# amisr/volumetricinterp

Hardware: AMD Instinct MI355X
Metric: fit+eval timesteps/sec (higher is better)
Workload: dtype f64

## Files before the change

### include/vinterp.h

```cpp
#ifndef VINTERP_H
#define VINTERP_H

#include <stddef.h>
#include <stdint.h>

#ifdef __cplusplus
extern "C" {
#endif

#define VI_ABI_VERSION 2

typedef enum vi_status {
    VI_OK = 0,
    VI_ERR_INVALID = -1,
    VI_ERR_HIP = -2,
    VI_ERR_ROCBLAS = -3,
    VI_ERR_ROCSOLVER = -4,
    VI_ERR_NOMEM = -5,
    VI_ERR_UNSUPPORTED = -6,
    VI_ERR_RCCL = -7
} vi_status;

typedef struct vi_ctx vi_ctx;
typedef struct vi_model vi_model;
// ... 65 lines not shown
int  vi_eval_track_f64(vi_model* model, int64_t Q, const double* d_lat, const double* d_lon, const double* d_alt,
                       const int32_t* d_rec, const double* d_w, int64_t R, const double* d_C,
                       const double* d_hull_eq, int32_t F, double hull_tol, double* d_out);
int  vi_eval_track_grad_f64(vi_model* model, int64_t Q, const double* d_lat, const double* d_lon, const double* d_alt,
                            const int32_t* d_rec, const double* d_w, int64_t R, const double* d_C,
                            const double* d_hull_eq, int32_t F, double hull_tol, int32_t frame, double* d_out);
int  vi_eval_slant_f64(vi_model* model, int64_t P, const double* d_a, const double* d_b, const int32_t* d_rec, const double* d_w,
                       int64_t R, const double* d_C, const double* d_hull_eq, int32_t F, double hull_tol, int32_t n,
                       const double* d_x, const double* d_wq, double* d_out, double* d_chord);
int  vi_eval_slant_basis_f64(vi_model* model, int64_t P, const double* d_a, const double* d_b, const double* d_hull_eq, int32_t F,
                             double hull_tol, int32_t n, const double* d_x, const double* d_wq, double* d_Y, double* d_chord);
int  vi_eval_basis_f64(vi_model* model, int64_t Q, const double* d_lat, const double* d_lon, const double* d_alt,
                       const double* d_hull_eq, int32_t F, double hull_tol, double* d_Y);
int  vi_eval_resident_f64(vi_model* model, int64_t Q, int64_t T, const double* d_Y, const double* d_C, double* d_out);
enum { VI_FRAME_MODEL = 0, VI_FRAME_ENU = 1 };
int  vi_eval_grad_basis_f64(vi_model* model, int64_t Q, const double* d_lat, const double* d_lon, const double* d_alt,
                            const double* d_hull_eq, int32_t F, double hull_tol, int32_t frame, double* d_G);
int  vi_eval_resident_err_f64(vi_model* model, int64_t Q, int64_t T, const double* d_Y, const double* d_dC, double* d_out);
int  vi_eval_resident_err_at_f64(vi_model* model, int64_t outer, int64_t L, int64_t inner, int64_t T, const double* d_Y,
                                 const double* d_dC, const int32_t* d_idx, double* d_out);
int  vi_eval_records_err_f64(vi_model* model, int64_t Q, const double* d_Y, const int32_t* d_rec, const double* d_w, int64_t R,
                             const double* d_dC, double* d_out);
int  vi_eval_track_err_f64(vi_model* model, int64_t Q, const double* d_lat, const double* d_lon, const double* d_alt,
                           const int32_t* d_rec, const double* d_w, int64_t R, const double* d_dC,
                           const double* d_hull_eq, int32_t F, double hull_tol, double* d_out);
int  vi_eval_slant_err_f64(vi_model* model, int64_t P, const double* d_a, const double* d_b, const int32_t* d_rec, const double* d_w,
                           int64_t R, const double* d_dC, const double* d_hull_eq, int32_t F, double hull_tol, int32_t n,
                           const double* d_x, const double* d_wq, double* d_out, double* d_chord);
int  vi_eval_resident_gradcov_f64(vi_model* model, int64_t Q, int64_t T, const double* d_G, const double* d_dC, double* d_out);
int  vi_eval_grad_cov_f64(vi_model* model, int64_t Q, const double* d_lat, const double* d_lon, const double* d_alt,
                          const double* d_dC, const double* d_hull_eq, int32_t F, double hull_tol, int32_t frame, double* d_out);
int  vi_eval_records_gradcov_f64(vi_model* model, int64_t Q, const double* d_G, const int32_t* d_rec, const double* d_w, int64_t R,
                                 const double* d_dC, double* d_out);
int  vi_eval_track_grad_cov_f64(vi_model* model, int64_t Q, const double* d_lat, const double* d_lon, const double* d_alt,
                                const int32_t* d_rec, const double* d_w, int64_t R, const double* d_dC,
                                const double* d_hull_eq, int32_t F, double hull_tol, int32_t frame, double* d_out);
int  vi_eval_hess_f64(vi_model* model, int64_t Q, const double* d_lat, const double* d_lon, const double* d_alt,
                      const double* d_C, const double* d_hull_eq, int32_t F, double hull_tol, int32_t frame, double* d_out);
int  vi_eval_hess_basis_f64(vi_model* model, int64_t Q, const double* d_lat, const double* d_lon, const double* d_alt,
                            const double* d_hull_eq, int32_t F, double hull_tol, int32_t frame, double* d_H);
int  vi_eval_peak_f64(vi_model* model, int64_t T, int64_t Q, const double* d_lat, const double* d_lon, const double* d_h0,
                      const double* d_lo, const double* d_hi, const double* d_C, const double* d_hull_eq, int32_t F,
                      double hull_tol, int32_t kind, int32_t max_iter, double tol, double* d_out, int32_t* d_status,
                      int32_t* d_iter);
int  vi_eval_level_f64(vi_model* model, int64_t T, int64_t Q, const double* d_lat, const double* d_lon, const double* d_ends,
                       const double* d_level, const double* d_C, const double* d_hull_eq, int32_t F, double hull_tol,
                       int32_t max_iter, double tol, double* d_out, int32_t* d_status, int32_t* d_iter);
int  vi_eval_ray_peak_f64(vi_model* model, int64_t T, int64_t P, const double* d_a, const double* d_b, const double* d_start,
                          const double* d_lo, const double* d_hi, const double* d_C, const double* d_hull_eq, int32_t F,
                          double hull_tol, int32_t kind, int32_t max_iter, double tol, double* d_out, int32_t* d_status,
                          int32_t* d_iter);
int  vi_eval_ray_level_f64(vi_model* model, int64_t T, int64_t P, const double* d_a, const double* d_b, const double* d_ends,
                           const double* d_level, const double* d_C, const double* d_hull_eq, int32_t F, double hull_tol,
                           int32_t max_iter, double tol, double* d_out, int32_t* d_status, int32_t* d_iter);
int  vi_eval_extremum_f64(vi_model* model, int64_t T, int64_t P, const double* d_x0, const double* d_radius, const double* d_C,
                          const double* d_hull_eq, int32_t F, double hull_tol, int32_t kind, double max_step, int32_t max_iter,
                          double tol, double* d_out, int32_t* d_status, int32_t* d_iter);
int    vi_eval_resident_peak_f64(vi_model* model, int64_t outer, int64_t L, int64_t inner, int64_t T, const double* d_Y,
                                 const double* d_C, int32_t kind, double* d_val, int32_t* d_idx, void* d_work, size_t work_bytes);
size_t vi_eval_resident_peak_work_bytes(vi_model* model, int64_t outer, int64_t L, int64_t inner, int64_t T);
int    vi_reduce_basis_f64(vi_model* model, int64_t outer, int64_t L, int64_t inner, const double* d_Y, const double* d_w,
                           double* d_Yr);
int    vi_eval_resident_cross_f64(vi_model* model, int64_t outer, int64_t L, int64_t inner, int64_t T, const double* d_Y,
                                  const double* d_C, const double* d_level, int32_t which, int32_t direction, int32_t* d_idx,
                                  void* d_work, size_t work_bytes);
int  vi_model_set_eval_precision(vi_model* model, int32_t chain_f32);
int  vi_ctx_set_eval_timing(vi_ctx* ctx, int32_t on);
int  vi_eval_kernel_ms(vi_ctx* ctx, double* ms);
int  vi_solve_timing(vi_ctx* ctx, int enable, int64_t* launches, int64_t* systems, int64_t* timed,
                     double* total_ms, double* max_ms);
int  vi_solve_rounds(vi_ctx* ctx, int64_t* rounds);
int  vi_eval_f64_host(vi_model* model, int64_t Q, const double* h_lat, const double* h_lon,
                      const double* h_alt, int64_t T, const double* h_C,
                      const double* h_hull_eq, int32_t F, double hull_tol, double* h_out);

int  vi_host_alloc(size_t bytes, void** out);
int  vi_host_free(void* p);

int  vi_normal_eq_f64(vi_ctx* ctx, int64_t T, int64_t P, int32_t N, const double* d_At,
                      const double* d_W, const double* d_b, double* d_AWA, double* d_y);

int  vi_form_system_f64(vi_ctx* ctx, int64_t B, int32_t N, const double* d_AWA, const int32_t* d_rec,
                        const double* d_alpha, const double* d_R, double* d_X);

int  vi_solve_trunc_f64(vi_ctx* ctx, int64_t B, int32_t N, double* d_X, const double* d_y,
                        const int32_t* d_rec, double rcond, double* d_C, int32_t* d_rank,
                        double pinv_rcond, double* d_H );

int  vi_chi2_f64(vi_ctx* ctx, int64_t B, int64_t P, int32_t N, const double* d_At, const double* d_C,
                 const int32_t* d_rec, const double* d_W, const double* d_b, double* d_chi2);

int  vi_cov_f64(vi_ctx* ctx, int64_t T, int32_t N, const double* d_H, const double* d_AWA, double* d_dC);

int  vi_warm_prepare_f64(vi_ctx* ctx, int64_t B, int32_t N, const double* d_AWA, const int32_t* d_rec,
                         const double* d_alpha0, const double* d_R, const double* d_y, double rcond,
                         double* d_C, int32_t* d_rank, double* d_V, double* d_D1, double* d_D2, double* d_yt);
int  vi_warm_solve_f64(vi_ctx* ctx, int64_t B, int32_t N, const double* d_D1, const double* d_D2,
                       const double* d_yt, const double* d_V, const int32_t* d_slot, const double* d_alpha,
                       double rcond, double* d_C, int32_t* d_rank, int32_t* d_sweeps );
int  vi_max_sweeps(void);

size_t vi_rotation_log_bytes(int32_t N);
int  vi_decompose_f64(vi_ctx* ctx, int64_t B, int32_t N, const double* d_AWA, const int32_t* d_rec,
                      const double* d_alpha0, const double* d_R, const double* d_y, double rcond, double* d_C,
                      int32_t* d_rank, void* d_log, int32_t* d_nround);
int  vi_warm_finish_f64(vi_ctx* ctx, int64_t B, int32_t N, const void* d_log, const int32_t* d_nround,
                        const double* d_AWA, const int32_t* d_rec, const double* d_R, const double* d_y,
                        double* d_V, double* d_D1, double* d_D2, double* d_yt);

int  vi_warm_rebase_f64(vi_ctx* ctx, int64_t B, int64_t nplain, int32_t N, const double* d_AWA, const double* d_R,
                        const double* d_y, const int32_t* d_rec, const int32_t* d_slot, const double* d_alpha, double rcond,
                        double* d_V, double* d_D1, double* d_D2, double* d_yt, double* d_C, int32_t* d_rank,
                        int32_t* d_sweeps );

int  vi_reg_floor_f64(vi_ctx* ctx, int64_t T, int32_t N, const double* d_AWA, const double* d_R, double* d_out);

int  vi_basis_solve_f64(vi_ctx* ctx, int64_t B, int32_t N, const double* d_AWA, const double* d_y,
                        const int32_t* d_rec, const int32_t* d_basis, const double* d_alpha, const double* d_V,
                        const double* d_D2, double rcond, double* d_C, int32_t* d_rank, int32_t* d_sweeps );

int  vi_warm_chi2_one_f64(vi_ctx* ctx, int32_t N, int64_t P, const double* d_D1, const double* d_D2,
                          const double* d_yt, const double* d_V, int32_t slot, double alpha, double rcond,
                          const double* d_At, int32_t rec, const double* d_W, const double* d_b,
                          double* d_scratch, double* h_chi2);

int  vi_brent_warm_f64(vi_ctx* ctx, int64_t ntask, int32_t N, int64_t P, double* d_D1, double* d_D2, double* d_yt,
                       double* d_V, const double* d_AWA, const double* d_R, const double* d_y, const double* h_rebase,
                       const double* d_At, const double* d_W, const double* d_b,
                       const int32_t* d_rec, const int32_t* d_slot, const double* d_xa, const double* d_xb,
                       const double* d_fa, const double* d_fb, const double* d_nu, double rcond, double* d_root,
                       double* d_other, int32_t* d_iters, int32_t* d_funcalls, int32_t* d_status);
int  vi_brent_warm_supported(int32_t N, int64_t P);
int  vi_brent_host_one_f64(vi_ctx* ctx, int32_t N, int64_t P, double* d_D1, double* d_D2, double* d_yt, double* d_V,
                           const double* d_AWA, const double* d_R, const double* d_y, const double* h_rebase,
                           const double* d_At, const double* d_W, const double* d_b, int32_t rec, int32_t slot,
                           double xa, double xb, double fa, double fb, double nu, double rcond, double* d_scratch,
                           double* h_out);
int  vi_exp10_f64(const double* x, double* out, int64_t n);

int  vi_gcv_terms_f64(vi_ctx* ctx, int64_t np, int64_t P, int32_t N, const double* d_At, const int32_t* d_pidx,
                      const double* d_AWA, const double* d_y, const double* d_W, const double* d_b,
                      double alpha, const double* d_R, double rcond, double* d_res);

int  vi_rccl_unique_id(char* out128);
int  vi_rccl_init(vi_ctx* ctx, int nranks, int rank, const char* id128);
int  vi_rccl_bcast_f64(vi_ctx* ctx, double* d_buf, int64_t count, int root);
int  vi_rccl_destroy(vi_ctx* ctx);

int  vi_eigvals_f64(vi_ctx* ctx, int64_t B, int32_t N, double* d_X, double* d_lam, int32_t* d_sweeps);

int  vi_qr_similarity_f64(vi_ctx* ctx, int64_t B, int32_t N, const double* d_X, const double* d_y, double* d_X1,
                          double* d_y1, double* d_Q);

int  vi_walk_form_f64(vi_ctx* ctx, int64_t B, int32_t N, const double* d_AWA, const int32_t* d_rec, const double* d_V,
                      const double* d_D2, const int32_t* d_basis, const double* d_y, const double* d_alpha, double* d_X,
                      double* d_scl, double* d_yt);

#ifdef __cplusplus
}
#endif
#endif
```

### volumetricinterp_amd/csrc/vi_qr.hip

```cpp
#include "vi_common.h"
#include "vi_solver.h"

#include <type_traits>

#ifdef VI_STAMPS
__device__ unsigned long long g_qr_stamps[8];
#define QR_STAMP(k)                                                        \
    do {                                                                   \
        const unsigned long long t_ = __builtin_readcyclecounter();        \
        if (blockIdx.x == 0 && threadIdx.x == 0) g_qr_stamps[k] += t_ - stamp_t; \
        stamp_t = __builtin_readcyclecounter();                            \
    } while (0)
#else
#define QR_STAMP(k)
#endif

namespace {

template <int CTRL, int ROWMASK>
__device__ __forceinline__ double dpp_mov(double v)
{
    const int lo = __builtin_amdgcn_update_dpp(__double2loint(v), __double2loint(v), CTRL, ROWMASK, 0xf, false);
    const int hi = __builtin_amdgcn_update_dpp(__double2hiint(v), __double2hiint(v), CTRL, ROWMASK, 0xf, false);
    return __hiloint2double(hi, lo);
}
__device__ __forceinline__ double octet_sum(double v)
{
    v += dpp_mov<0xB1, 0xf>(v);
    v += dpp_mov<0x4E, 0xf>(v);
    v += dpp_mov<0x141, 0xf>(v);
    return v;
}
__device__ __forceinline__ double wave_max_octets(double v)
{
    v = fmax(v, dpp_mov<0x118, 0xf>(v));
    v = fmax(v, dpp_mov<0x142, 0xa>(v));
    v = fmax(v, dpp_mov<0x143, 0xc>(v));
    const int lo = __builtin_amdgcn_readlane(__double2loint(v), 63);
    const int hi = __builtin_amdgcn_readlane(__double2hiint(v), 63);
    return __hiloint2double(hi, lo);
}
__device__ __forceinline__ double wave_sum(double v)
{
    v += dpp_mov<0xB1, 0xf>(v);
    v += dpp_mov<0x4E, 0xf>(v);
    v += dpp_mov<0x141, 0xf>(v);
    v += dpp_mov<0x140, 0xf>(v);
    {
        const int lo = __builtin_amdgcn_update_dpp(0, __double2loint(v), 0x142, 0xa, 0xf, false);
        const int hi = __builtin_amdgcn_update_dpp(0, __double2hiint(v), 0x142, 0xa, 0xf, false);
        v += __hiloint2double(hi, lo);
    }
    {
        const int lo = __builtin_amdgcn_update_dpp(0, __double2loint(v), 0x143, 0xc, 0xf, false);
        const int hi = __builtin_amdgcn_update_dpp(0, __double2hiint(v), 0x143, 0xc, 0xf, false);
        v += __hiloint2double(hi, lo);
    }
    const int lo = __builtin_amdgcn_readlane(__double2loint(v), 63);
    const int hi = __builtin_amdgcn_readlane(__double2hiint(v), 63);
    return __hiloint2double(hi, lo);
}

__device__ __forceinline__ void lds_barrier()
{
    asm volatile("s_waitcnt lgkmcnt(0)\n\ts_barrier" ::: "memory");
}

__device__ __forceinline__ double qr_rsqrt(double x)
{
    const double y = __builtin_amdgcn_rsq(x);
    const double e = fma(-x * y, y, 1.0);
    return fma(y, e * fma(0.375, e, 0.5), y);
}
__device__ __forceinline__ double qr_rcp(double x)
{
    double y = __builtin_amdgcn_rcp(x);
    y = fma(y, fma(-x, y, 1.0), y);
    y = fma(y, fma(-x, y, 1.0), y);
    return y;
}

__host__ __device__ __forceinline__ int hh_off(int k, int NR)
{
    const int B = k >> 3;
    return 8 * NR * B - 32 * B * (B - 1) + (k & 7) * (NR - 8 * B);
}
__host__ __device__ __forceinline__ size_t hh_doubles(int N, int NR)
{
    return (size_t)hh_off(N, NR) + (size_t)N;
}

template <int I, int E, class F>
__device__ __forceinline__ bool static_up(F&& f)
{
    if constexpr (I < E) {
        if (f(std::integral_constant<int, I>{})) return true;
        return static_up<I + 1, E>(f);
    }
    return false;
}
template <int I, class F>
__device__ __forceinline__ void static_down(F&& f)
{
    if constexpr (I >= 0) {
        f(std::integral_constant<int, I>{});
        static_down<I - 1>(f);
    }
}

template <int RT, int I0>
__device__ __forceinline__ void reflect2(double (&a0)[RT], double (&a1)[RT], const double* __restrict__ vl, double tau)
{
    double d0 = 0.0, d1 = 0.0;
#pragma unroll
    for (int i = I0; i < RT; ++i) {
        const double v = vl[8 * i];
        d0 = fma(v, a0[i], d0);
        d1 = fma(v, a1[i], d1);
    }
    const double w0 = tau * octet_sum(d0), w1 = tau * octet_sum(d1);
    asm volatile("" ::: "memory");
#pragma unroll
    for (int i = I0; i < RT; ++i) {
        const double v = vl[8 * i];
        a0[i] = fma(-w0, v, a0[i]);
        a1[i] = fma(-w1, v, a1[i]);
    }
}

template <int RT>
__global__ __launch_bounds__(RT <= 8 ? 320 : 640) void k_qr_sim(
    int N, const double* __restrict__ X, const double* __restrict__ y, const int* __restrict__ rec, double* X1,
    double* __restrict__ y1, double* __restrict__ hh, int64_t hh_stride, double* __restrict__ Rscr)
{
    extern __shared__ __align__(16) unsigned char lds_raw[];
    constexpr int NR = 8 * RT;
    double* vcur = reinterpret_cast<double*>(lds_raw);
    double* Vst = vcur + 2 * NR;
    const int nvst = hh_off(N, NR);
    double* taus = Vst + nvst;
    double* redv = taus + N;
    int* redi = reinterpret_cast<int*>(redv + 16);

    const int tid = threadIdx.x, lane = tid & 63, wave = tid >> 6, nw = blockDim.x >> 6;
    const int l = tid & 7, c0 = (tid >> 3) << 1, c1 = c0 + 1;
    const int64_t sys = blockIdx.x;
    const double* Xs = X + sys * (int64_t)N * N;
    const double* ys = y + (int64_t)(rec ? rec[sys] : sys) * N;
    double* Rs = Rscr + sys * (int64_t)N * N;
    const bool m0 = c0 < N, m1 = c1 < N;

#ifdef VI_STAMPS
    unsigned long long stamp_t = __builtin_readcyclecounter();
#endif
    double a0[RT], a1[RT];
#pragma unroll
    for (int i = 0; i < RT; ++i) {
        const int r = 8 * i + l;
        a0[i] = (r < N) ? (m0 ? Xs[(int64_t)(r > c0 ? r : c0) * N + (r > c0 ? c0 : r)] : (c0 == N ? ys[r] : 0.0)) : 0.0;
        a1[i] = (r < N) ? (m1 ? Xs[(int64_t)(r > c1 ? r : c1) * N + (r > c1 ? c1 : r)] : (c1 == N ? ys[r] : 0.0)) : 0.0;
    }
    for (int r = tid; r < 2 * NR; r += blockDim.x) vcur[r] = 0.0;
    for (int k = tid; k < N; k += blockDim.x) taus[k] = 0.0;
    for (int e = tid; e < nvst; e += blockDim.x) Vst[e] = 0.0;
    double n0 = 0.0, n1 = 0.0;
#pragma unroll
    for (int i = 0; i < RT; ++i) {
        n0 = fma(a0[i], a0[i], n0);
        n1 = fma(a1[i], a1[i], n1);
    }
    n0 = octet_sum(n0);
    n1 = octet_sum(n1);
    bool done0 = !m0, done1 = !m1;
    int K = 0;
    __syncthreads();
    QR_STAMP(0);
    static_up<0, RT>([&](auto I0c) -> bool {
        constexpr int I0 = decltype(I0c)::value;
        for (int lk = 0; lk < 8; ++lk) {
            const int k = 8 * I0 + lk;
            if (k >= N - 1) return true;
            const double v0 = done0 ? -1.0 : n0, v1 = done1 ? -1.0 : n1;
            const double cv = v1 > v0 ? v1 : v0;
            const int ci = v1 > v0 ? c1 : c0;
            const double wm = wave_max_octets(cv);
            const unsigned long long hit = __ballot(cv >= 0.0 && cv == wm);
            const int first = hit ? (__ffsll((long long)hit) - 1) : 0;
            const int wi = __builtin_amdgcn_readlane(ci, first);
            if (lane == 0) {
                redv[wave] = hit ? wm : -1.0;
                redi[wave] = wi;
            }
            lds_barrier();
            QR_STAMP(1);
            double pmax = redv[0];
            int p = redi[0];
#pragma unroll
            for (int w = 1; w < 10; ++w) {
                const double ov = w < nw ? redv[w] : -1.0;
                const int oi = w < nw ? redi[w] : 0;
                const bool take = ov > pmax;
                pmax = take ? ov : pmax;
                p = take ? oi : p;
            }
            if (!(pmax > 0.0)) return true;
            double* vb = vcur + (k & 1) * NR + l;
            if ((p >> 1) == (tid >> 3)) {
                const bool second = p & 1;
                const double xk = __shfl(second ? a1[I0] : a0[I0], (lane & ~7) | lk);
                const double ri_ = qr_rsqrt(pmax);
                const double nx = pmax * ri_;
                const double alpha = -copysign(nx, xk);
                const double vk = xk - alpha;
                const double tau = ri_ * qr_rcp(nx + fabs(xk));
                double* vs = Vst + hh_off(k, NR) - 8 * I0 + l;
#pragma unroll
                for (int i = I0; i < RT; ++i) {
                    const double x = second ? a1[i] : a0[i];
                    const double v = (i == I0 && l == lk) ? vk : x;
                    vb[8 * i] = v;
                    vs[8 * i] = v;
                }
                if (l == 0) taus[k] = tau;
                done0 = done0 || !second;
                done1 = done1 || second;
            }
            lds_barrier();
            QR_STAMP(2);
            K = k + 1;
            const double tau = taus[k];
            double d0 = 0.0, d1 = 0.0;
#pragma unroll
            for (int i = I0; i < RT; ++i) {
                const double v = vb[8 * i];
                d0 = fma(v, a0[i], d0);
                d1 = fma(v, a1[i], d1);
            }
            const double w0 = tau * octet_sum(d0), w1 = tau * octet_sum(d1);
            asm volatile("" ::: "memory");
            n0 = 0.0;
            n1 = 0.0;
#pragma unroll
            for (int i = I0; i < RT; ++i) {
                const double v = vb[8 * i];
                a0[i] = fma(-w0, v, a0[i]);
                a1[i] = fma(-w1, v, a1[i]);
                if (i == I0) {
                    if (l == lk) {
                        if (m0) Rs[(int64_t)k * N + c0] = a0[i];
                        if (m1) Rs[(int64_t)k * N + c1] = a1[i];
                        a0[i] = 0.0;
                        a1[i] = 0.0;
                    }
                }
                n0 = fma(a0[i], a0[i], n0);
                n1 = fma(a1[i], a1[i], n1);
            }
            n0 = octet_sum(n0);
            n1 = octet_sum(n1);
            QR_STAMP(3);
        }
        return false;
    });
    __syncthreads();
#pragma unroll
    for (int i = 0; i < RT; ++i) {
        const int r = 8 * i + l;
        if (r >= K && r < N) {
            if (m0) Rs[(int64_t)r * N + c0] = a0[i];
            if (m1) Rs[(int64_t)r * N + c1] = a1[i];
        }
    }
    {
        double* hs = hh + sys * hh_stride;
        for (int e = tid; e < nvst + N; e += blockDim.x) hs[e] = Vst[e];
    }
    __syncthreads();
    QR_STAMP(4);
#pragma unroll
    for (int i = 0; i < RT; ++i) {
        const int r = 8 * i + l;
        a0[i] = (r < N) ? (m0 ? Rs[(int64_t)c0 * N + r] : (c0 == N ? ys[r] : 0.0)) : 0.0;
        a1[i] = (r < N) ? (m1 ? Rs[(int64_t)c1 * N + r] : (c1 == N ? ys[r] : 0.0)) : 0.0;
    }
    QR_STAMP(5);
    static_up<0, RT>([&](auto I0c) -> bool {
        constexpr int I0 = decltype(I0c)::value;
        for (int k = 8 * I0; k < 8 * I0 + 8; ++k) {
            if (k >= K) return true;
            reflect2<RT, I0>(a0, a1, Vst + hh_off(k, NR) - 8 * I0 + l, taus[k]);
        }
        return false;
    });
    QR_STAMP(6);
    double* Xo = X1 + sys * (int64_t)N * N;
#pragma unroll
    for (int i = 0; i < RT; ++i) {
        const int r = 8 * i + l;
        if (r < N) {
            if (m0) Xo[(int64_t)c0 * N + r] = a0[i];
            else if (c0 == N) y1[sys * N + r] = a0[i];
            if (m1) Xo[(int64_t)c1 * N + r] = a1[i];
            else if (c1 == N) y1[sys * N + r] = a1[i];
        }
    }
}

template <int EPL>
__global__ __launch_bounds__(256) void k_qr_back_vec(int N, int NR, const double* __restrict__ hh, int64_t hh_stride,
                                                     double* __restrict__ C)
{
    extern __shared__ __align__(16) unsigned char lds_raw[];
    double* Vst = reinterpret_cast<double*>(lds_raw);
    const int nvst = hh_off(N, NR);
    const double* taus = Vst + nvst;
    const int tid = threadIdx.x;
    const int64_t sys = blockIdx.x;
    const double* hs = hh + sys * hh_stride;
    for (int e = tid; e < nvst + N; e += blockDim.x) Vst[e] = hs[e];
    __syncthreads();
    if (tid >= 64) return;
    double* c = C + sys * N;
    double x[EPL];
#pragma unroll
    for (int j = 0; j < EPL; ++j) {
        const int r = tid + 64 * j;
        x[j] = r < N ? c[r] : 0.0;
    }
    for (int k = N - 2; k >= 0; --k) {
        const double tau = taus[k];
        if (tau == 0.0) continue;
        const double* vk = Vst + hh_off(k, NR) - 8 * (k >> 3);
        const int r0 = 8 * (k >> 3);
        double v[EPL];
        double dot = 0.0;
#pragma unroll
        for (int j = 0; j < EPL; ++j) {
            const int r = tid + 64 * j;
            v[j] = (r >= r0 && r < NR) ? vk[r] : 0.0;
            dot = fma(v[j], x[j], dot);
        }
        const double w = tau * wave_sum(dot);
#pragma unroll
        for (int j = 0; j < EPL; ++j) x[j] = fma(-w, v[j], x[j]);
    }
#pragma unroll
    for (int j = 0; j < EPL; ++j) {
        const int r = tid + 64 * j;
        if (r < N) c[r] = x[j];
    }
}

template <int RT>
__global__ __launch_bounds__(RT <= 8 ? 320 : 640) void k_qr_back_mat(int N, const double* __restrict__ hh, int64_t hh_stride,
                                                                     double* __restrict__ V)
{
    extern __shared__ __align__(16) unsigned char lds_raw[];
    double* Vst = reinterpret_cast<double*>(lds_raw);
    constexpr int NR = 8 * RT;
    const int nvst = hh_off(N, NR);
    double* taus = Vst + nvst;
    const int tid = threadIdx.x, l = tid & 7, c0 = (tid >> 3) << 1, c1 = c0 + 1;
    const int64_t sys = blockIdx.x;
    const double* hs = hh + sys * hh_stride;
    for (int e = tid; e < nvst + N; e += blockDim.x) Vst[e] = hs[e];
    __syncthreads();
    if (c0 >= N) return;
    double* Vs = V + sys * (int64_t)N * N;
    const bool m1 = c1 < N;
    double a0[RT], a1[RT];
#pragma unroll
    for (int i = 0; i < RT; ++i) {
        const int r = 8 * i + l;
        a0[i] = r < N ? Vs[(int64_t)c0 * N + r] : 0.0;
        a1[i] = (r < N && m1) ? Vs[(int64_t)c1 * N + r] : 0.0;
    }
    static_down<RT - 1>([&](auto I0c) {
        constexpr int I0 = decltype(I0c)::value;
        for (int k = 8 * I0 + 7; k >= 8 * I0; --k) {
            const double tau = k < N ? taus[k] : 0.0;
            if (tau != 0.0) reflect2<RT, I0>(a0, a1, Vst + hh_off(k, NR) - 8 * I0 + l, tau);
        }
    });
#pragma unroll
    for (int i = 0; i < RT; ++i) {
        const int r = 8 * i + l;
        if (r < N) {
            Vs[(int64_t)c0 * N + r] = a0[i];
            if (m1) Vs[(int64_t)c1 * N + r] = a1[i];
        }
    }
}

}
#ifdef VI_STAMPS
extern "C" int vi_debug_qr_stamps(double* out, int reset)
{
    unsigned long long h[8];
    if (hipMemcpyFromSymbol(h, HIP_SYMBOL(g_qr_stamps), sizeof(h)) != hipSuccess) return -1;
    for (int i = 0; i < 8; ++i) out[i] = (double)h[i];
    if (reset) {
        memset(h, 0, sizeof(h));
        if (hipMemcpyToSymbol(HIP_SYMBOL(g_qr_stamps), h, sizeof(h)) != hipSuccess) return -1;
    }
    return 0;
}
#endif
namespace {

int qr_rt(int N)
{
    const int need = (N + 7) / 8;
    const int opts[] = {4, 6, 8, 12, 18};
    for (int o : opts)
        if (need <= o) return o;
    return 0;
}

size_t qr_lds_bytes(int N)
{
    return (size_t)2 * 8 * qr_rt(N) * 8 + (hh_doubles(N, 8 * qr_rt(N)) + 16) * 8 + 16 * 4;
}

}

bool vi_qr_supported(int N) { return N >= 8 && qr_rt(N) > 0 && qr_lds_bytes(N) <= 159 * 1024; }
size_t vi_qr_hh_bytes(int N) { return hh_doubles(N, 8 * qr_rt(N)) * sizeof(double); }

int vi_qr_precond(vi_ctx* c, int64_t B, int N, const double* d_X, const double* d_y, const int* d_rec, double* d_X1,
                  double* d_y1, double* d_hh, double* d_scr, int64_t hh_stride)
{
    if (hh_stride <= 0) hh_stride = (int64_t)(vi_qr_hh_bytes(N) / sizeof(double));
    const int rt = qr_rt(N);
    const int threads = ((8 * ((N + 2) / 2) + 63) / 64) * 64;
    const size_t shm = qr_lds_bytes(N);
#define VI_QR(R)                                                                                                            \
    do {                                                                                                                    \
        VI_HIP(hipFuncSetAttribute((const void*)k_qr_sim<R>, hipFuncAttributeMaxDynamicSharedMemorySize, (int)shm));        \
        hipLaunchKernelGGL(k_qr_sim<R>, dim3((unsigned)B), dim3(threads), shm, c->stream, N, d_X, d_y, d_rec, d_X1, d_y1,   \
                           d_hh, hh_stride, d_scr);                                                                         \
    } while (0)
    switch (rt) {
    case 4: VI_QR(4); break;
    case 6: VI_QR(6); break;
    case 8: VI_QR(8); break;
    case 12: VI_QR(12); break;
    case 18: VI_QR(18); break;
    default: vi_set_error("vi_qr_precond: N=%d unsupported", N); return VI_ERR_UNSUPPORTED;
    }
#undef VI_QR
    VI_HIP(hipGetLastError());
    return VI_OK;
}

int vi_qr_back_vec(vi_ctx* c, int64_t B, int N, const double* d_hh, double* d_C, int64_t hh_stride)
{
    if (hh_stride <= 0) hh_stride = (int64_t)(vi_qr_hh_bytes(N) / sizeof(double));
    const size_t shm = vi_qr_hh_bytes(N);
#define VI_QV(E)                                                                                                            \
    do {                                                                                                                    \
        VI_HIP(hipFuncSetAttribute((const void*)k_qr_back_vec<E>, hipFuncAttributeMaxDynamicSharedMemorySize, (int)shm));   \
        hipLaunchKernelGGL(k_qr_back_vec<E>, dim3((unsigned)B), dim3(256), shm, c->stream, N, 8 * qr_rt(N), d_hh, hh_stride, d_C);        \
    } while (0)
    if (N <= 64) VI_QV(1);
    else if (N <= 128) VI_QV(2);
    else VI_QV(3);
#undef VI_QV
    VI_HIP(hipGetLastError());
    return VI_OK;
}

int vi_qr_back_mat(vi_ctx* c, int64_t B, int N, const double* d_hh, double* d_V, int64_t hh_stride)
{
    if (hh_stride <= 0) hh_stride = (int64_t)(vi_qr_hh_bytes(N) / sizeof(double));
    const int rt = qr_rt(N);
    const int threads = ((8 * ((N + 1) / 2) + 63) / 64) * 64;
    const size_t shm = vi_qr_hh_bytes(N);
#define VI_QB(R)                                                                                                            \
    do {                                                                                                                    \
        VI_HIP(hipFuncSetAttribute((const void*)k_qr_back_mat<R>, hipFuncAttributeMaxDynamicSharedMemorySize, (int)shm));   \
        hipLaunchKernelGGL(k_qr_back_mat<R>, dim3((unsigned)B), dim3(threads), shm, c->stream, N, d_hh, hh_stride, d_V);    \
    } while (0)
    switch (rt) {
    case 4: VI_QB(4); break;
    case 6: VI_QB(6); break;
    case 8: VI_QB(8); break;
    case 12: VI_QB(12); break;
    case 18: VI_QB(18); break;
    default: vi_set_error("vi_qr_back_mat: N=%d unsupported", N); return VI_ERR_UNSUPPORTED;
    }
#undef VI_QB
    VI_HIP(hipGetLastError());
    return VI_OK;
}

extern "C" int vi_qr_similarity_f64(vi_ctx* c, int64_t B, int32_t N, const double* d_X, const double* d_y, double* d_X1,
                                    double* d_y1, double* d_Q)
{
    VI_REQUIRE(c && d_X && d_y && d_X1 && d_y1 && d_Q, "null argument");
    VI_REQUIRE(B >= 0 && N > 0, "bad size");
    if (B == 0) return VI_OK;
    if (!vi_qr_supported(N)) {
        vi_set_error("vi_qr_similarity_f64: N=%d outside the range of the register-resident QR", N);
        return VI_ERR_UNSUPPORTED;
    }
    VI_HIP(hipSetDevice(c->device));
    double *hhp, *scr;
    int rc = ws_carve(c, [&](ws_carver& w) {
        hhp = w.take<double>((size_t)B * (vi_qr_hh_bytes(N) / sizeof(double)));
        scr = w.take<double>((size_t)B * N * N);
    });
    if (rc != VI_OK) return rc;
    if ((rc = vi_qr_precond(c, B, N, d_X, d_y, nullptr, d_X1, d_y1, hhp, scr, 0)) != VI_OK) return rc;
    std::vector<double> eye((size_t)N * N, 0.0);
    for (int i = 0; i < N; ++i) eye[(size_t)i * N + i] = 1.0;
    for (int64_t b = 0; b < B; ++b)
        VI_HIP(hipMemcpyAsync(d_Q + b * (int64_t)N * N, eye.data(), eye.size() * sizeof(double), hipMemcpyHostToDevice, c->stream));
    VI_HIP(hipStreamSynchronize(c->stream));
    return vi_qr_back_mat(c, B, N, hhp, d_Q, 0);
}
```

### volumetricinterp_amd/fitengine.py

```python
import ctypes as C
import functools
import math
import os
import threading

import numpy as np

from . import _lib
from . import alpha_search

EPS = float(np.finfo(np.float64).eps)

_lib._sig('vi_normal_eq_f64', C.c_int, _lib.VOIDP, C.c_int64, C.c_int64, C.c_int32, _lib.VOIDP, _lib.VOIDP,
          _lib.VOIDP, _lib.VOIDP, _lib.VOIDP)
_lib._sig('vi_form_system_f64', C.c_int, _lib.VOIDP, C.c_int64, C.c_int32, _lib.VOIDP, _lib.VOIDP, _lib.VOIDP,
          _lib.VOIDP, _lib.VOIDP)
_lib._sig('vi_solve_trunc_f64', C.c_int, _lib.VOIDP, C.c_int64, C.c_int32, _lib.VOIDP, _lib.VOIDP, _lib.VOIDP,
          C.c_double, _lib.VOIDP, _lib.VOIDP, C.c_double, _lib.VOIDP)
_lib._sig('vi_chi2_f64', C.c_int, _lib.VOIDP, C.c_int64, C.c_int64, C.c_int32, _lib.VOIDP, _lib.VOIDP, _lib.VOIDP,
          _lib.VOIDP, _lib.VOIDP, _lib.VOIDP)
_lib._sig('vi_cov_f64', C.c_int, _lib.VOIDP, C.c_int64, C.c_int32, _lib.VOIDP, _lib.VOIDP, _lib.VOIDP)
_lib._sig('vi_warm_prepare_f64', C.c_int, _lib.VOIDP, C.c_int64, C.c_int32, _lib.VOIDP, _lib.VOIDP, _lib.VOIDP, _lib.VOIDP,
          _lib.VOIDP, C.c_double, _lib.VOIDP, _lib.VOIDP, _lib.VOIDP, _lib.VOIDP, _lib.VOIDP, _lib.VOIDP)
_lib._sig('vi_warm_solve_f64', C.c_int, _lib.VOIDP, C.c_int64, C.c_int32, _lib.VOIDP, _lib.VOIDP, _lib.VOIDP, _lib.VOIDP,
          _lib.VOIDP, _lib.VOIDP, C.c_double, _lib.VOIDP, _lib.VOIDP, _lib.VOIDP)
_lib._sig('vi_basis_solve_f64', C.c_int, _lib.VOIDP, C.c_int64, C.c_int32, _lib.VOIDP, _lib.VOIDP, _lib.VOIDP, _lib.VOIDP,
          _lib.VOIDP, _lib.VOIDP, _lib.VOIDP, C.c_double, _lib.VOIDP, _lib.VOIDP, _lib.VOIDP)
_lib._sig('vi_max_sweeps', C.c_int)
_lib._sig('vi_cold_max_sweeps', C.c_int, C.c_int32)
_lib._sig('vi_brent_warm_f64', C.c_int, _lib.VOIDP, C.c_int64, C.c_int32, C.c_int64, *([_lib.VOIDP] * 18), C.c_double,
          *([_lib.VOIDP] * 5))
_lib._sig('vi_exp10_f64', C.c_int, _lib.VOIDP, _lib.VOIDP, C.c_int64)
_lib._sig('vi_reg_floor_f64', C.c_int, _lib.VOIDP, C.c_int64, C.c_int32, _lib.VOIDP, _lib.VOIDP, _lib.VOIDP)
_lib._sig('vi_rotation_log_bytes', C.c_size_t, C.c_int32)
_lib._sig('vi_decompose_f64', C.c_int, _lib.VOIDP, C.c_int64, C.c_int32, _lib.VOIDP, _lib.VOIDP, _lib.VOIDP, _lib.VOIDP,
          _lib.VOIDP, C.c_double, _lib.VOIDP, _lib.VOIDP, _lib.VOIDP, _lib.VOIDP)
_lib._sig('vi_warm_finish_f64', C.c_int, _lib.VOIDP, C.c_int64, C.c_int32, _lib.VOIDP, _lib.VOIDP, _lib.VOIDP, _lib.VOIDP,
          _lib.VOIDP, _lib.VOIDP, _lib.VOIDP, _lib.VOIDP, _lib.VOIDP, _lib.VOIDP)
_lib._sig('vi_warm_rebase_f64', C.c_int, _lib.VOIDP, C.c_int64, C.c_int64, C.c_int32, _lib.VOIDP, _lib.VOIDP, _lib.VOIDP, _lib.VOIDP,
          _lib.VOIDP, _lib.VOIDP, C.c_double, _lib.VOIDP, _lib.VOIDP, _lib.VOIDP, _lib.VOIDP, _lib.VOIDP, _lib.VOIDP,
          _lib.VOIDP)
_lib._sig('vi_warm_chi2_one_f64', C.c_int, _lib.VOIDP, C.c_int32, C.c_int64, _lib.VOIDP, _lib.VOIDP, _lib.VOIDP, _lib.VOIDP,
          C.c_int32, C.c_double, C.c_double, _lib.VOIDP, C.c_int32, _lib.VOIDP, _lib.VOIDP, _lib.VOIDP,
          C.POINTER(C.c_double))
_lib._sig('vi_gcv_terms_f64', C.c_int, _lib.VOIDP, C.c_int64, C.c_int64, C.c_int32, _lib.VOIDP, _lib.VOIDP, _lib.VOIDP,
          _lib.VOIDP, _lib.VOIDP, _lib.VOIDP, C.c_double, _lib.VOIDP, C.c_double, _lib.VOIDP)
_lib._sig('vi_eigvals_f64', C.c_int, _lib.VOIDP, C.c_int64, C.c_int32, _lib.VOIDP, _lib.VOIDP, _lib.VOIDP)
_lib._sig('vi_qr_similarity_f64', C.c_int, _lib.VOIDP, C.c_int64, C.c_int32, _lib.VOIDP, _lib.VOIDP, _lib.VOIDP, _lib.VOIDP,
          _lib.VOIDP)
_lib._sig('vi_walk_form_f64', C.c_int, _lib.VOIDP, C.c_int64, C.c_int32, *([_lib.VOIDP] * 10))
_lib._sig('vi_brent_host_one_f64', C.c_int, _lib.VOIDP, C.c_int32, C.c_int64, *([_lib.VOIDP] * 11), C.c_int32, C.c_int32,
          C.c_double, C.c_double, C.c_double, C.c_double, C.c_double, C.c_double, _lib.VOIDP, _lib.VOIDP)
_lib._sig('vi_brent_warm_supported', C.c_int, C.c_int32, C.c_int64)
_lib.EXPORTS += ['vi_brent_warm_supported', 'vi_brent_host_one_f64', 'vi_brent_warm_f64', 'vi_exp10_f64', 'vi_max_sweeps', 'vi_cold_max_sweeps', 'vi_qr_similarity_f64', 'vi_walk_form_f64', 'vi_rotation_log_bytes', 'vi_decompose_f64', 'vi_warm_finish_f64', 'vi_warm_rebase_f64', 'vi_reg_floor_f64', 'vi_basis_solve_f64', 'vi_warm_chi2_one_f64', 'vi_gcv_terms_f64', 'vi_warm_prepare_f64', 'vi_warm_solve_f64', 'vi_eigvals_f64', 'vi_normal_eq_f64', 'vi_form_system_f64', 'vi_solve_trunc_f64', 'vi_chi2_f64', 'vi_cov_f64']



def _flag(name, default='1'):
    return os.environ.get('VINTERP_' + name, default) != '0'


MAX_BATCH = 8192


class _View(object):

    def __init__(self, parent, offset_elems):
        self._parent = parent
        self.dtype = parent.dtype
        self.ptr = parent.offset_ptr(offset_elems)

    def offset_ptr(self, nelem):
        return C.c_void_p(self.ptr.value + int(nelem) * self.dtype.itemsize)


class FitEngine(object):
    RESIDENT_BUFFERS = ('W', 'b', 'Wref', 'bref', 'AWA', 'y')

    def __init__(self, ctx, At_dev, P, N, reg_matrices, regularization_list, scratch_of=None):
        self._scratch_of = scratch_of
        self.ctx = ctx
        self.At = At_dev
        self.P, self.N = int(P), int(N)
        self.regularization_list = list(regularization_list)
        self.R = {}
        self._R_host = {}
        for name in self.regularization_list:
            M = np.ascontiguousarray(reg_matrices[name], dtype=np.float64)
            if M.shape != (self.N, self.N):
                raise ValueError('regularisation matrix %r has shape %r, expected %r' % (name, M.shape, (N, N)))
            if not np.all(np.isfinite(M)):
                raise ValueError('array must not contain infs or NaNs')
            self.R[name] = ctx.to_device(M)
            self._R_host[name] = M
        self._bufs = {}
        self.T = 0
        self._ref_rec = None
        self._subs = None
        self._bounds = [0, 0]
        self._same_below = {}
        self._walk_cache = {}
        self._warm_slot = {}
        self._spec_slot = {}
        self._basis_x = {}
        self.stats = dict(solves=0, launches=0)

    @classmethod
    def from_host_basis(cls, ctx, A, reg_matrices, regularization_list):
        A = np.asarray(A, dtype=np.float64)
        if A.ndim != 2:
            raise ValueError('A must be (npoints, nbasis)')
        if not np.all(np.isfinite(A)):
            raise ValueError('array must not contain infs or NaNs')
        At = ctx.to_device(np.ascontiguousarray(A.T))
        return cls(ctx, At, A.shape[0], A.shape[1], reg_matrices, regularization_list)

    def _buf(self, name, shape, dtype=np.float64):
        if self._scratch_of is not None and name not in self.RESIDENT_BUFFERS:
            return self._scratch_of._buf(name, shape, dtype)
        n = int(np.prod(shape, dtype=np.int64))
        cur = self._bufs.get(name)
        if cur is None or cur.size < n or cur.dtype != np.dtype(dtype):
            if cur is not None:
                cur.free()
            cur = _lib.DeviceArray(self.ctx, (max(n, 1),), dtype)
            self._bufs[name] = cur
        return cur

    def _count(self, key, n=1):
        self.stats[key] = self.stats.get(key, 0) + n

    def upload_records(self, W, b):
        W = np.ascontiguousarray(W, dtype=np.float64)
        b = np.ascontiguousarray(b, dtype=np.float64)
        if W.shape != b.shape or W.ndim != 2 or W.shape[1] != self.P:
            raise ValueError('W, b must both be (T, %d)' % self.P)
        self.T = T = W.shape[0]
        self.dW = self._buf('W', W.shape).upload(W) if T else None
        self.db = self._buf('b', b.shape).upload(b) if T else None
        K = self.pipelines()
        self._bounds = [(T * k) // K for k in range(K + 1)]
        self._ref_host = [(np.mean(W[lo:hi], axis=0, keepdims=True), np.mean(b[lo:hi], axis=0, keepdims=True))
                          for lo, hi in zip(self._bounds[:-1], self._bounds[1:])] if T else []
        self._ref_rec = None
        if T:
            self._set_reference(*(self._ref_host[0] if K == 1 else (np.mean(W, axis=0, keepdims=True),
                                                                    np.mean(b, axis=0, keepdims=True))))

    def _set_reference(self, Wref, bref):
        self._ref_rec = None
        if self.T and self.shared_walk_enabled():
            self.dWref = self._buf('Wref', (1, self.P)).upload(Wref)
            self.dbref = self._buf('bref', (1, self.P)).upload(bref)
            self._ref_rec = self.T

    def adopt_records(self, dW, db, T, Wref, bref):
        self.T = int(T)
        self._close_subs()
        self.dW, self.db = dW, db
        self._bounds = [0, self.T]
        self._ref_host = [(Wref, bref)]
        self._set_reference(Wref, bref)

    PIPELINE_MIN_RECORDS = 75

    def pipelines(self):
        if getattr(self, '_no_pipeline', False) or not self.warm_enabled():
            return 1
        k = os.environ.get('VINTERP_PIPELINES')
        if k is not None:
            return max(1, min(int(k), max(1, self.T)))
        try:
            queues = int(_lib.HW_QUEUES_REQUESTED)
        except ValueError:
            queues = 4
        self.stats['hw_queues_requested'] = queues
        return int(max(1, min(4 if queues >= 8 else 2, self.T // self.PIPELINE_MIN_RECORDS)))

    def form_normal_equations(self):
        T, N = self.T, self.N
        self.dAWA = self._buf('AWA', (T + 1, N, N))
        self.dy = self._buf('y', (T + 1, N))
        if T:
            _lib.check(_lib.lib.vi_normal_eq_f64(self.ctx.handle, T, self.P, N, self.At.ptr, self.dW.ptr, self.db.ptr,
                                                 self.dAWA.ptr, self.dy.ptr), 'vi_normal_eq_f64')
            if self._ref_rec is not None:
                _lib.check(_lib.lib.vi_normal_eq_f64(self.ctx.handle, 1, self.P, N, self.At.ptr, self.dWref.ptr,
                                                     self.dbref.ptr, self.dAWA.offset_ptr(T * N * N),
                                                     self.dy.offset_ptr(T * N)), 'vi_normal_eq_f64')

    def load_records(self, W, b):
        self.upload_records(W, b)
        self.form_normal_equations()

    def normal_equations(self):
        T, N = self.T, self.N
        return self.dAWA.download((T, N, N)), self.dy.download((T, N))

    def _solve_chunk(self, rec, alphas, want_H, tag):
        B, N = len(rec), self.N
        drec = self._buf(tag + 'rec', (B,), np.int32).upload(rec)
        dX = self._buf(tag + 'X', (B, N, N))
        first = True
        for name in self.regularization_list:
            a = np.ascontiguousarray(alphas[name], dtype=np.float64)
            dal = self._buf(tag + 'alpha_' + name, (B,)).upload(a)
            _lib.check(_lib.lib.vi_form_system_f64(self.ctx.handle, B, N, self.dAWA.ptr if first else None,
# ... 950 lines not shown
```

Measured before the change: 3723.

## Pack four systems per block in QR back-vec and prefetch reflectors from global

The vector back-application kernel no longer stages the reflector set into shared memory. Each 64-lane wavefront now handles its own system, four per block. Reflector columns and taus are read straight from global memory through an 8-deep register prefetch ring, with scheduling barriers so the loads overlap the dot/update work. A timing entry point (vi_qr_back_f64) and extra cycle stamps are added for profiling. The risks are higher register pressure from the prefetch ring and scattered global reads in place of a coalesced LDS fill.

```diff
diff --git a/include/vinterp.h b/include/vinterp.h
--- a/include/vinterp.h
+++ b/include/vinterp.h
@@ -241,6 +241,9 @@
 int  vi_qr_similarity_f64(vi_ctx* ctx, int64_t B, int32_t N, const double* d_X, const double* d_y, double* d_X1,
                           double* d_y1, double* d_Q);
 
+int  vi_qr_back_f64(vi_ctx* ctx, int64_t B, int32_t N, const double* d_X, const double* d_y, int64_t hh_stride,
+                    double* d_Q, double* d_C, double* d_V, double* h_ms);
+
 int  vi_walk_form_f64(vi_ctx* ctx, int64_t B, int32_t N, const double* d_AWA, const int32_t* d_rec, const double* d_V,
                       const double* d_D2, const int32_t* d_basis, const double* d_y, const double* d_alpha, double* d_X,
                       double* d_scl, double* d_yt);
diff --git a/volumetricinterp_amd/csrc/vi_qr.hip b/volumetricinterp_amd/csrc/vi_qr.hip
--- a/volumetricinterp_amd/csrc/vi_qr.hip
+++ b/volumetricinterp_amd/csrc/vi_qr.hip
@@ -4,7 +4,7 @@
 #include <type_traits>
 
 #ifdef VI_STAMPS
-__device__ unsigned long long g_qr_stamps[8];
+__device__ unsigned long long g_qr_stamps[16];
 #define QR_STAMP(k)                                                        \
     do {                                                                   \
         const unsigned long long t_ = __builtin_readcyclecounter();        \
@@ -306,49 +306,77 @@
     }
 }
 
+constexpr int QR_AHEAD = 8;
 template <int EPL>
-__global__ __launch_bounds__(256) void k_qr_back_vec(int N, int NR, const double* __restrict__ hh, int64_t hh_stride,
+__global__ __launch_bounds__(256) void k_qr_back_vec(int64_t B, int N, int NR, const double* __restrict__ hh, int64_t hh_stride,
                                                      double* __restrict__ C)
 {
-    extern __shared__ __align__(16) unsigned char lds_raw[];
-    double* Vst = reinterpret_cast<double*>(lds_raw);
-    const int nvst = hh_off(N, NR);
-    const double* taus = Vst + nvst;
-    const int tid = threadIdx.x;
-    const int64_t sys = blockIdx.x;
+    const int lane = threadIdx.x & 63;
+    const int64_t sys = 4 * (int64_t)blockIdx.x + (threadIdx.x >> 6);
+    if (sys >= B) return;
+#ifdef VI_STAMPS
+    unsigned long long stamp_t = __builtin_readcyclecounter();
+#endif
     const double* hs = hh + sys * hh_stride;
-    for (int e = tid; e < nvst + N; e += blockDim.x) Vst[e] = hs[e];
-    __syncthreads();
-    if (tid >= 64) return;
+    const double* taus = hs + hh_off(N, NR);
     double* c = C + sys * N;
     double x[EPL];
 #pragma unroll
     for (int j = 0; j < EPL; ++j) {
-        const int r = tid + 64 * j;
+        const int r = lane + 64 * j;
         x[j] = r < N ? c[r] : 0.0;
     }
-    for (int k = N - 2; k >= 0; --k) {
-        const double tau = taus[k];
-        if (tau == 0.0) continue;
-        const double* vk = Vst + hh_off(k, NR) - 8 * (k >> 3);
+    double wv[QR_AHEAD][EPL], wt[QR_AHEAD];
+    auto fetch = [&](int k, double (&v)[EPL], double& t) {
+        k = k < 0 ? 0 : k;
         const int r0 = 8 * (k >> 3);
-        double v[EPL];
-        double dot = 0.0;
+        const double* vk = hs + hh_off(k, NR) - r0;
 #pragma unroll
         for (int j = 0; j < EPL; ++j) {
-            const int r = tid + 64 * j;
-            v[j] = (r >= r0 && r < NR) ? vk[r] : 0.0;
-            dot = fma(v[j], x[j], dot);
-        }
-        const double w = tau * wave_sum(dot);
-#pragma unroll
-        for (int j = 0; j < EPL; ++j) x[j] = fma(-w, v[j], x[j]);
-    }
+            const int r = lane + 64 * j;
+            v[j] = vk[r < r0 ? r0 : (r < NR ? r : NR - 1)];
+        }
+        t = taus[k];
+    };
+#pragma unroll
+    for (int s = 0; s < QR_AHEAD; ++s) {
+        fetch(N - 2 - s, wv[s], wt[s]);
+        __builtin_amdgcn_sched_barrier(0);
+    }
+    QR_STAMP(8);
+    for (int kb = N - 2; kb >= 0; kb -= QR_AHEAD) {
+#pragma unroll
+        for (int s = 0; s < QR_AHEAD; ++s) {
+            const int k = kb - s;
+            const int r0 = 8 * (k >> 3);
+            const double tk = __hiloint2double(__builtin_amdgcn_readfirstlane(__double2hiint(wt[s])),
+                                               __builtin_amdgcn_readfirstlane(__double2loint(wt[s])));
+            const double tau = k >= 0 ? tk : 0.0;
+            double v[EPL];
+#pragma unroll
+            for (int j = 0; j < EPL; ++j) {
+                const int r = lane + 64 * j;
+                v[j] = (r >= r0 && r < NR) ? wv[s][j] : 0.0;
+            }
+            fetch(k - QR_AHEAD, wv[s], wt[s]);
+            __builtin_amdgcn_sched_barrier(0);
+            if (tau != 0.0) {
+                double dot = 0.0;
+#pragma unroll
+                for (int j = 0; j < EPL; ++j) dot = fma(v[j], x[j], dot);
+                const double w = tau * wave_sum(dot);
+#pragma unroll
+                for (int j = 0; j < EPL; ++j) x[j] = fma(-w, v[j], x[j]);
+            }
+        }
+    }
+    QR_STAMP(9);
 #pragma unroll
     for (int j = 0; j < EPL; ++j) {
-        const int r = tid + 64 * j;
+        const int r = lane + 64 * j;
         if (r < N) c[r] = x[j];
     }
+    QR_STAMP(10);
 }
 
 template <int RT>
@@ -363,8 +391,12 @@
     const int tid = threadIdx.x, l = tid & 7, c0 = (tid >> 3) << 1, c1 = c0 + 1;
     const int64_t sys = blockIdx.x;
     const double* hs = hh + sys * hh_stride;
+#ifdef VI_STAMPS
+    unsigned long long stamp_t = __builtin_readcyclecounter();
+#endif
     for (int e = tid; e < nvst + N; e += blockDim.x) Vst[e] = hs[e];
     __syncthreads();
+    QR_STAMP(11);
     if (c0 >= N) return;
     double* Vs = V + sys * (int64_t)N * N;
     const bool m1 = c1 < N;
@@ -375,6 +407,7 @@
         a0[i] = r < N ? Vs[(int64_t)c0 * N + r] : 0.0;
         a1[i] = (r < N && m1) ? Vs[(int64_t)c1 * N + r] : 0.0;
     }
+    QR_STAMP(12);
     static_down<RT - 1>([&](auto I0c) {
         constexpr int I0 = decltype(I0c)::value;
         for (int k = 8 * I0 + 7; k >= 8 * I0; --k) {
@@ -382,6 +415,7 @@
             if (tau != 0.0) reflect2<RT, I0>(a0, a1, Vst + hh_off(k, NR) - 8 * I0 + l, tau);
         }
     });
+    QR_STAMP(13);
 #pragma unroll
     for (int i = 0; i < RT; ++i) {
         const int r = 8 * i + l;
@@ -390,15 +424,16 @@
             if (m1) Vs[(int64_t)c1 * N + r] = a1[i];
         }
     }
+    QR_STAMP(14);
 }
 
 }
 #ifdef VI_STAMPS
 extern "C" int vi_debug_qr_stamps(double* out, int reset)
 {
-    unsigned long long h[8];
+    unsigned long long h[16];
     if (hipMemcpyFromSymbol(h, HIP_SYMBOL(g_qr_stamps), sizeof(h)) != hipSuccess) return -1;
-    for (int i = 0; i < 8; ++i) out[i] = (double)h[i];
+    for (int i = 0; i < 16; ++i) out[i] = (double)h[i];
     if (reset) {
         memset(h, 0, sizeof(h));
         if (hipMemcpyToSymbol(HIP_SYMBOL(g_qr_stamps), h, sizeof(h)) != hipSuccess) return -1;
@@ -456,12 +491,9 @@
 int vi_qr_back_vec(vi_ctx* c, int64_t B, int N, const double* d_hh, double* d_C, int64_t hh_stride)
 {
     if (hh_stride <= 0) hh_stride = (int64_t)(vi_qr_hh_bytes(N) / sizeof(double));
-    const size_t shm = vi_qr_hh_bytes(N);
 #define VI_QV(E)                                                                                                            \
-    do {                                                                                                                    \
-        VI_HIP(hipFuncSetAttribute((const void*)k_qr_back_vec<E>, hipFuncAttributeMaxDynamicSharedMemorySize, (int)shm));   \
-        hipLaunchKernelGGL(k_qr_back_vec<E>, dim3((unsigned)B), dim3(256), shm, c->stream, N, 8 * qr_rt(N), d_hh, hh_stride, d_C);        \
-    } while (0)
+    hipLaunchKernelGGL(k_qr_back_vec<E>, dim3((unsigned)((B + 3) / 4)), dim3(256), 0, c->stream, B, N, 8 * qr_rt(N), d_hh,  \
+                       hh_stride, d_C)
     if (N <= 64) VI_QV(1);
     else if (N <= 128) VI_QV(2);
     else VI_QV(3);
@@ -519,3 +551,54 @@
     VI_HIP(hipStreamSynchronize(c->stream));
     return vi_qr_back_mat(c, B, N, hhp, d_Q, 0);
 }
+
+extern "C" int vi_qr_back_f64(vi_ctx* c, int64_t B, int32_t N, const double* d_X, const double* d_y, int64_t hh_stride,
+                              double* d_Q, double* d_C, double* d_V, double* h_ms)
+{
+    VI_REQUIRE(c && d_X && d_y, "null argument");
+    VI_REQUIRE(B >= 0 && N > 0, "bad size");
+    if (B == 0) return VI_OK;
+    if (!vi_qr_supported(N)) {
+        vi_set_error("vi_qr_back_f64: N=%d outside the range of the register-resident QR", N);
+        return VI_ERR_UNSUPPORTED;
+    }
+    const int64_t hhd = (int64_t)(vi_qr_hh_bytes(N) / sizeof(double));
+    if (hh_stride <= 0) hh_stride = hhd;
+    VI_REQUIRE(hh_stride >= hhd, "hh_stride shorter than a reflector set");
+    VI_HIP(hipSetDevice(c->device));
+    double *hhp, *scr, *X1, *y1;
+    int rc = ws_carve(c, [&](ws_carver& w) {
+        hhp = w.take<double>((size_t)B * hh_stride);
+        scr = w.take<double>((size_t)B * N * N);
+        X1 = w.take<double>((size_t)B * N * N);
+        y1 = w.take<double>((size_t)B * N);
+    });
+    if (rc != VI_OK) return rc;
+    hipEvent_t ev[6] = {};
+    for (auto& e : ev) VI_HIP(hipEventCreate(&e));
+    VI_HIP(hipEventRecord(ev[0], c->stream));
+    if ((rc = vi_qr_precond(c, B, N, d_X, d_y, nullptr, X1, y1, hhp, scr, hh_stride)) != VI_OK) return rc;
+    VI_HIP(hipEventRecord(ev[1], c->stream));
+    if (d_Q) {
+        std::vector<double> eye((size_t)N * N, 0.0);
+        for (int i = 0; i < N; ++i) eye[(size_t)i * N + i] = 1.0;
+        for (int64_t b = 0; b < B; ++b)
+            VI_HIP(hipMemcpyAsync(d_Q + b * (int64_t)N * N, eye.data(), eye.size() * sizeof(double), hipMemcpyHostToDevice, c->stream));
+        VI_HIP(hipStreamSynchronize(c->stream));
+        if ((rc = vi_qr_back_mat(c, B, N, hhp, d_Q, hh_stride)) != VI_OK) return rc;
+    }
+    VI_HIP(hipEventRecord(ev[2], c->stream));
+    if (d_C && (rc = vi_qr_back_vec(c, B, N, hhp, d_C, hh_stride)) != VI_OK) return rc;
+    VI_HIP(hipEventRecord(ev[3], c->stream));
+    VI_HIP(hipEventRecord(ev[4], c->stream));
+    if (d_V && (rc = vi_qr_back_mat(c, B, N, hhp, d_V, hh_stride)) != VI_OK) return rc;
+    VI_HIP(hipEventRecord(ev[5], c->stream));
+    VI_HIP(hipStreamSynchronize(c->stream));
+    for (int i = 0; i < 3; ++i) {
+        float ms = 0.f;
+        VI_HIP(hipEventElapsedTime(&ms, ev[2 * i], ev[2 * i + 1]));
+        if (h_ms) h_ms[i] = (i == 0 || (i == 1 ? d_C : d_V) != nullptr) ? (double)ms : 0.0;
+    }
+    for (auto& e : ev) VI_HIP(hipEventDestroy(e));
+    return VI_OK;
+}
diff --git a/volumetricinterp_amd/fitengine.py b/volumetricinterp_amd/fitengine.py
--- a/volumetricinterp_amd/fitengine.py
+++ b/volumetricinterp_amd/fitengine.py
@@ -48,11 +48,13 @@
 _lib._sig('vi_eigvals_f64', C.c_int, _lib.VOIDP, C.c_int64, C.c_int32, _lib.VOIDP, _lib.VOIDP, _lib.VOIDP)
 _lib._sig('vi_qr_similarity_f64', C.c_int, _lib.VOIDP, C.c_int64, C.c_int32, _lib.VOIDP, _lib.VOIDP, _lib.VOIDP, _lib.VOIDP,
           _lib.VOIDP)
+_lib._sig('vi_qr_back_f64', C.c_int, _lib.VOIDP, C.c_int64, C.c_int32, _lib.VOIDP, _lib.VOIDP, C.c_int64, _lib.VOIDP,
+          _lib.VOIDP, _lib.VOIDP, C.POINTER(C.c_double))
 _lib._sig('vi_walk_form_f64', C.c_int, _lib.VOIDP, C.c_int64, C.c_int32, *([_lib.VOIDP] * 10))
 _lib._sig('vi_brent_host_one_f64', C.c_int, _lib.VOIDP, C.c_int32, C.c_int64, *([_lib.VOIDP] * 11), C.c_int32, C.c_int32,
           C.c_double, C.c_double, C.c_double, C.c_double, C.c_double, C.c_double, _lib.VOIDP, _lib.VOIDP)
 _lib._sig('vi_brent_warm_supported', C.c_int, C.c_int32, C.c_int64)
-_lib.EXPORTS += ['vi_brent_warm_supported', 'vi_brent_host_one_f64', 'vi_brent_warm_f64', 'vi_exp10_f64', 'vi_max_sweeps', 'vi_cold_max_sweeps', 'vi_qr_similarity_f64', 'vi_walk_form_f64', 'vi_rotation_log_bytes', 'vi_decompose_f64', 'vi_warm_finish_f64', 'vi_warm_rebase_f64', 'vi_reg_floor_f64', 'vi_basis_solve_f64', 'vi_warm_chi2_one_f64', 'vi_gcv_terms_f64', 'vi_warm_prepare_f64', 'vi_warm_solve_f64', 'vi_eigvals_f64', 'vi_normal_eq_f64', 'vi_form_system_f64', 'vi_solve_trunc_f64', 'vi_chi2_f64', 'vi_cov_f64']
+_lib.EXPORTS += ['vi_brent_warm_supported', 'vi_brent_host_one_f64', 'vi_brent_warm_f64', 'vi_exp10_f64', 'vi_max_sweeps', 'vi_cold_max_sweeps', 'vi_qr_similarity_f64', 'vi_qr_back_f64', 'vi_walk_form_f64', 'vi_rotation_log_bytes', 'vi_decompose_f64', 'vi_warm_finish_f64', 'vi_warm_rebase_f64', 'vi_reg_floor_f64', 'vi_basis_solve_f64', 'vi_warm_chi2_one_f64', 'vi_gcv_terms_f64', 'vi_warm_prepare_f64', 'vi_warm_solve_f64', 'vi_eigvals_f64', 'vi_normal_eq_f64', 'vi_form_system_f64', 'vi_solve_trunc_f64', 'vi_chi2_f64', 'vi_cov_f64']
 
 
 
```

Result: no change. 3749, median of 5 (+0.7%).
